# debbiemarkslab/EVcouplings

Measured on NVIDIA H100. Metric: PLM gradient evals/s as N*L^2*q cell-ops/s, higher is better.
Workload: dtype f32 parameters/accumulation; tensor-core products as bf16 hi+lo pairs (16 mantissa bits)

## Files before the change

evcouplings_b200/csrc/plm_tc.cu:

```cuda
#include <cuda.h>
#include <cuda_bf16.h>

#include <stdlib.h>

#include <algorithm>

#include "common.cuh"
#include "internal.h"

namespace evc {

constexpr int TC_BM = 128;
constexpr int TC_BN = 192;
constexpr int TC_BK = 64;
constexpr int TC_MAX_STAGES = 8;
constexpr int TC_A_BYTES = TC_BM * TC_BK * 2;
constexpr int TC_B_BYTES = TC_BN * TC_BK * 2;
constexpr int TC_SMEM_LIMIT = 232448;
constexpr int TC_SMEM_HEAD = 2048;
constexpr int TC_THREADS = 384;
constexpr int TC_CONSUMERS = 256;
constexpr int TC_K_CHUNK = 32;
constexpr int TC_MAX_KSPLIT = 8;
constexpr int TC_REG_PRODUCER = 40;
// ... 104 lines not shown
          "+f"(d[56]), "+f"(d[57]), "+f"(d[58]), "+f"(d[59]), "+f"(d[60]), "+f"(d[61]), "+f"(d[62]), "+f"(d[63]),
          "+f"(d[64]), "+f"(d[65]), "+f"(d[66]), "+f"(d[67]), "+f"(d[68]), "+f"(d[69]), "+f"(d[70]), "+f"(d[71]),
          "+f"(d[72]), "+f"(d[73]), "+f"(d[74]), "+f"(d[75]), "+f"(d[76]), "+f"(d[77]), "+f"(d[78]), "+f"(d[79]),
          "+f"(d[80]), "+f"(d[81]), "+f"(d[82]), "+f"(d[83]), "+f"(d[84]), "+f"(d[85]), "+f"(d[86]), "+f"(d[87]),
          "+f"(d[88]), "+f"(d[89]), "+f"(d[90]), "+f"(d[91]), "+f"(d[92]), "+f"(d[93]), "+f"(d[94]), "+f"(d[95])
        : "l"(da), "l"(db), "r"(scale_d));
}
template <>
__device__ __forceinline__ void wgmma_bf16<176>(float *d, uint64_t da, uint64_t db, uint32_t scale_d)
{
    asm volatile(
        "{\n.reg .pred p;\n"
        "setp.ne.b32 p, %90, 0;\n"
        "wgmma.mma_async.sync.aligned.m64n176k16.f32.bf16.bf16 "
        "{"
        "%0, %1, %2, %3, %4, %5, %6, %7, %8, %9, %10, %11, %12, %13, %14, %15, "
        "%16, %17, %18, %19, %20, %21, %22, %23, %24, %25, %26, %27, %28, %29, %30, %31, "
        "%32, %33, %34, %35, %36, %37, %38, %39, %40, %41, %42, %43, %44, %45, %46, %47, "
        "%48, %49, %50, %51, %52, %53, %54, %55, %56, %57, %58, %59, %60, %61, %62, %63, "
        "%64, %65, %66, %67, %68, %69, %70, %71, %72, %73, %74, %75, %76, %77, %78, %79, "
        "%80, %81, %82, %83, %84, %85, %86, %87"
        "}, %88, %89, p, 1, 1, 0, 0;\n}\n"
        : "+f"(d[0]), "+f"(d[1]), "+f"(d[2]), "+f"(d[3]), "+f"(d[4]), "+f"(d[5]), "+f"(d[6]), "+f"(d[7]),
          "+f"(d[8]), "+f"(d[9]), "+f"(d[10]), "+f"(d[11]), "+f"(d[12]), "+f"(d[13]), "+f"(d[14]), "+f"(d[15]),
          "+f"(d[16]), "+f"(d[17]), "+f"(d[18]), "+f"(d[19]), "+f"(d[20]), "+f"(d[21]), "+f"(d[22]), "+f"(d[23]),
          "+f"(d[24]), "+f"(d[25]), "+f"(d[26]), "+f"(d[27]), "+f"(d[28]), "+f"(d[29]), "+f"(d[30]), "+f"(d[31]),
          "+f"(d[32]), "+f"(d[33]), "+f"(d[34]), "+f"(d[35]), "+f"(d[36]), "+f"(d[37]), "+f"(d[38]), "+f"(d[39]),
          "+f"(d[40]), "+f"(d[41]), "+f"(d[42]), "+f"(d[43]), "+f"(d[44]), "+f"(d[45]), "+f"(d[46]), "+f"(d[47]),
          "+f"(d[48]), "+f"(d[49]), "+f"(d[50]), "+f"(d[51]), "+f"(d[52]), "+f"(d[53]), "+f"(d[54]), "+f"(d[55]),
          "+f"(d[56]), "+f"(d[57]), "+f"(d[58]), "+f"(d[59]), "+f"(d[60]), "+f"(d[61]), "+f"(d[62]), "+f"(d[63]),
          "+f"(d[64]), "+f"(d[65]), "+f"(d[66]), "+f"(d[67]), "+f"(d[68]), "+f"(d[69]), "+f"(d[70]), "+f"(d[71]),
          "+f"(d[72]), "+f"(d[73]), "+f"(d[74]), "+f"(d[75]), "+f"(d[76]), "+f"(d[77]), "+f"(d[78]), "+f"(d[79]),
          "+f"(d[80]), "+f"(d[81]), "+f"(d[82]), "+f"(d[83]), "+f"(d[84]), "+f"(d[85]), "+f"(d[86]), "+f"(d[87])
        : "l"(da), "l"(db), "r"(scale_d));
}

__device__ __forceinline__ void wgmma_sp_bf16_192(float *d, const uint4 &a, uint32_t e, uint64_t db, uint32_t scale_d)
{
    asm volatile(
        "{\n.reg .pred p;\n"
        "setp.ne.b32 p, %102, 0;\n"
        "wgmma.mma_async.sp.sync.aligned.m64n192k32.f32.bf16.bf16 "
        "{"
        "%0, %1, %2, %3, %4, %5, %6, %7, %8, %9, %10, %11, %12, %13, %14, %15, "
        "%16, %17, %18, %19, %20, %21, %22, %23, %24, %25, %26, %27, %28, %29, %30, %31, "
        "%32, %33, %34, %35, %36, %37, %38, %39, %40, %41, %42, %43, %44, %45, %46, %47, "
        "%48, %49, %50, %51, %52, %53, %54, %55, %56, %57, %58, %59, %60, %61, %62, %63, "
        "%64, %65, %66, %67, %68, %69, %70, %71, %72, %73, %74, %75, %76, %77, %78, %79, "
        "%80, %81, %82, %83, %84, %85, %86, %87, %88, %89, %90, %91, %92, %93, %94, %95"
        "}, {%96, %97, %98, %99}, %100, %101, 0, p, 1, 1, 0;\n}\n"
        : "+f"(d[0]), "+f"(d[1]), "+f"(d[2]), "+f"(d[3]), "+f"(d[4]), "+f"(d[5]), "+f"(d[6]), "+f"(d[7]),
          "+f"(d[8]), "+f"(d[9]), "+f"(d[10]), "+f"(d[11]), "+f"(d[12]), "+f"(d[13]), "+f"(d[14]), "+f"(d[15]),
          "+f"(d[16]), "+f"(d[17]), "+f"(d[18]), "+f"(d[19]), "+f"(d[20]), "+f"(d[21]), "+f"(d[22]), "+f"(d[23]),
          "+f"(d[24]), "+f"(d[25]), "+f"(d[26]), "+f"(d[27]), "+f"(d[28]), "+f"(d[29]), "+f"(d[30]), "+f"(d[31]),
          "+f"(d[32]), "+f"(d[33]), "+f"(d[34]), "+f"(d[35]), "+f"(d[36]), "+f"(d[37]), "+f"(d[38]), "+f"(d[39]),
          "+f"(d[40]), "+f"(d[41]), "+f"(d[42]), "+f"(d[43]), "+f"(d[44]), "+f"(d[45]), "+f"(d[46]), "+f"(d[47]),
          "+f"(d[48]), "+f"(d[49]), "+f"(d[50]), "+f"(d[51]), "+f"(d[52]), "+f"(d[53]), "+f"(d[54]), "+f"(d[55]),
          "+f"(d[56]), "+f"(d[57]), "+f"(d[58]), "+f"(d[59]), "+f"(d[60]), "+f"(d[61]), "+f"(d[62]), "+f"(d[63]),
          "+f"(d[64]), "+f"(d[65]), "+f"(d[66]), "+f"(d[67]), "+f"(d[68]), "+f"(d[69]), "+f"(d[70]), "+f"(d[71]),
          "+f"(d[72]), "+f"(d[73]), "+f"(d[74]), "+f"(d[75]), "+f"(d[76]), "+f"(d[77]), "+f"(d[78]), "+f"(d[79]),
          "+f"(d[80]), "+f"(d[81]), "+f"(d[82]), "+f"(d[83]), "+f"(d[84]), "+f"(d[85]), "+f"(d[86]), "+f"(d[87]),
          "+f"(d[88]), "+f"(d[89]), "+f"(d[90]), "+f"(d[91]), "+f"(d[92]), "+f"(d[93]), "+f"(d[94]), "+f"(d[95])
        : "r"(a.x), "r"(a.y), "r"(a.z), "r"(a.w), "l"(db), "r"(e), "r"(scale_d));
}

__device__ __forceinline__ uint4 lds128(uint32_t addr)
{
    uint4 v;
    asm volatile("ld.shared.v4.u32 {%0, %1, %2, %3}, [%4];" : "=r"(v.x), "=r"(v.y), "=r"(v.z), "=r"(v.w) : "r"(addr));
    return v;
}
__device__ __forceinline__ uint32_t lds32(uint32_t addr)
{
    uint32_t v;
    asm volatile("ld.shared.u32 %0, [%1];" : "=r"(v) : "r"(addr));
    return v;
}
__device__ __forceinline__ uint32_t cluster_ctarank()
{
    uint32_t r;
    asm volatile("mov.u32 %0, %%cluster_ctarank;" : "=r"(r));
    return r;
}
__device__ __forceinline__ void cluster_sync()
{
    asm volatile("barrier.cluster.arrive.release;\nbarrier.cluster.wait.acquire;" ::: "memory");
}
__device__ __forceinline__ void mbar_arrive_cluster(uint64_t *bar, uint32_t rank)
{
    uint32_t remote;
    asm volatile("mapa.shared::cluster.u32 %0, %1, %2;" : "=r"(remote) : "r"(smem_u32(bar)), "r"(rank));
    asm volatile("mbarrier.arrive.shared::cluster.b64 _, [%0];" ::"r"(remote) : "memory");
}
__device__ __forceinline__ void tma_load_2d_multicast(void *smem_dst, const CUtensorMap *tmap, int c0, int c1,
                                                      uint64_t *bar, uint16_t mask, uint64_t policy)
{
    asm volatile(
        "cp.async.bulk.tensor.2d.shared::cluster.global.mbarrier::complete_tx::bytes.multicast::cluster.L2::cache_hint"
        " [%0], [%1, {%4, %5}], [%2], %3, %6;"
        ::"r"(smem_u32(smem_dst)), "l"(reinterpret_cast<uint64_t>(tmap)), "r"(smem_u32(bar)), "h"(mask), "r"(c0),
        "r"(c1), "l"(policy)
        : "memory");
}

template <int N>
__device__ __forceinline__ void wgmma_kblock(float *acc, uint64_t a, uint64_t b, uint64_t a2, uint64_t b2, bool two,
                                             bool overwrite)
{
#pragma unroll
    for (int k = 0; k < TC_BK / 16; k++) {
        const uint64_t koff = (uint64_t)((k * 16 * 2) >> 4);
        wgmma_bf16<N>(acc, a + koff, b + koff, (overwrite && k == 0) ? 0u : 1u);
        if (two) wgmma_bf16<N>(acc, a2 + koff, b2 + koff, 1u);
    }
}

template <int N>
__device__ __forceinline__ void tc_mainloop(float *acc, uint64_t *full, uint64_t *empty, int &s, uint32_t &ph,
                                            int n_stages, int stage_bytes, int kb0, int kb1, uint64_t desc0,
                                            uint64_t off_a, uint64_t off_b, uint64_t off_a2, uint64_t off_b2, bool two)
{
    int prev = -1;
    for (int kb = kb0; kb < kb1; kb++) {
        mbar_wait_bounded(&full[s], ph);
        wgmma_fence();
        const uint64_t d = desc0 + (uint64_t)((s * stage_bytes) >> 4);
        wgmma_kblock<N>(acc, d + off_a, d + off_b, d + off_a2, d + off_b2, two, kb == kb0);
        wgmma_commit();
        wgmma_wait<1>();
        if (prev >= 0) mbar_arrive(&empty[prev]);
        prev = s;
        if (++s == n_stages) { s = 0; ph ^= 1u; }
    }
    wgmma_wait<0>();
    fence_regs<N / 2>(acc);
    if (prev >= 0) mbar_arrive(&empty[prev]);
}

__device__ __forceinline__ void decode_tile(int tile, int m_tiles, int n_tiles, int mgroup, int &m_tile, int &n_tile)
{
    const int full = (m_tiles / mgroup) * mgroup * n_tiles;
    if (tile < full) {
        const int per = mgroup * n_tiles;
        const int g = tile / per, r = tile - g * per;
        n_tile = r / mgroup;
        m_tile = g * mgroup + (r - n_tile * mgroup);
    } else {
        const int rem = m_tiles % mgroup, r = tile - full;
        n_tile = r / rem;
        m_tile = (m_tiles / mgroup) * mgroup + (r - n_tile * rem);
    }
}

struct TcSmem {
    uint64_t *full, *empty;
    unsigned char *ring;
};
__device__ __forceinline__ TcSmem tc_smem_layout(unsigned char *smem_dyn)
{
    unsigned char *base = reinterpret_cast<unsigned char *>((reinterpret_cast<uintptr_t>(smem_dyn) + 1023) &
                                                            ~static_cast<uintptr_t>(1023));
    TcSmem l;
    l.full = reinterpret_cast<uint64_t *>(base);
    l.empty = l.full + TC_MAX_STAGES;
    l.ring = base + 1024;
    return l;
// ... 23 lines not shown
    extern __shared__ unsigned char smem_dyn[];
    const TcSmem l = tc_smem_layout(smem_dyn);
    const int tiles = m_tiles * n_tiles;
    const int slice = (int)blockIdx.x / tiles;
    int m_tile, n_tile;
    decode_tile((int)blockIdx.x - slice * tiles, m_tiles, n_tiles, mgroup, m_tile, n_tile);
    const int kb_per = (num_kb + ksplit - 1) / ksplit;
    const int kb_begin = slice * kb_per, kb_end = min(num_kb, kb_begin + kb_per);
    tc_init_barriers(l, n_stages);

    if (threadIdx.x < 128) {
        setmaxnreg_dec<TC_REG_PRODUCER>();
        if (threadIdx.x == 0) {
            int s = 0;
            uint32_t ph = 0;
            for (int kb = kb_begin; kb < kb_end; kb++) {
                mbar_wait_bounded(&l.empty[s], ph ^ 1u);
                unsigned char *st = l.ring + s * stage_bytes;
                mbar_expect_tx(&l.full[s], (uint32_t)stage_bytes);
                tma_load_2d(st, &tm0, kb * TC_BK, m_tile * TC_BM, &l.full[s]);
                tma_load_2d(st + BYTES0, &tm1, kb * TC_BK, n_tile * TC_BN, &l.full[s]);
                if (!SINGLE) tma_load_2d(st + BYTES0 + BYTES1, &tm2, kb * TC_BK, n_tile * TC_BN, &l.full[s]);
                if (++s == n_stages) { s = 0; ph ^= 1u; }
            }
        }
    } else {
        setmaxnreg_inc<TC_REG_CONSUMER>();
        const int cw = (threadIdx.x >> 7) - 1;
        constexpr uint64_t OFF1 = (uint64_t)(BYTES0 >> 4), OFF2 = (uint64_t)((BYTES0 + BYTES1) >> 4);
        const uint64_t arow = (uint64_t)((cw * 64 * TC_BK * 2) >> 4);
        const uint64_t desc0 = make_desc_sw128(l.ring);
        float acc[TC_BN / 2], sum[TC_BN / 2];
#pragma unroll
        for (int u = 0; u < TC_BN / 2; u++) acc[u] = 0.f;
        const int n_chunks = (kb_end - kb_begin + k_chunk - 1) / k_chunk;
        int s = 0;
        uint32_t ph = 0;
        for (int c = 0; c < n_chunks; c++) {
            const int kb0 = kb_begin + c * k_chunk, kb1 = min(kb_end, kb0 + k_chunk);
            tc_mainloop<TC_BN>(acc, l.full, l.empty, s, ph, n_stages, stage_bytes, kb0, kb1, desc0,
                               arow, OFF1, arow, OFF2, !SINGLE);
#pragma unroll
            for (int u = 0; u < TC_BN / 2; u++) sum[u] = (c == 0) ? acc[u] : sum[u] + acc[u];
        }
        const int t = threadIdx.x & 127;
        const int64_t row = (int64_t)m_tile * TC_BM + cw * 64 + (t >> 5) * 16 + ((t & 31) >> 2);
        float *out = D + slice * plane + row * ldd + (int64_t)n_tile * TC_BN + 2 * (t & 3);
        if (ACC && slice < acc_planes) {
#pragma unroll
            for (int c8 = 0; c8 < TC_BN / 8; c8++) {
                float2 *p0 = reinterpret_cast<float2 *>(out + 8 * c8);
                float2 *p1 = reinterpret_cast<float2 *>(out + 8 * ldd + 8 * c8);
                const float2 v0 = __ldcs(p0), v1 = __ldcs(p1);
                __stcs(p0, make_float2(v0.x + sum[4 * c8], v0.y + sum[4 * c8 + 1]));
                __stcs(p1, make_float2(v1.x + sum[4 * c8 + 2], v1.y + sum[4 * c8 + 3]));
            }
            return;
        }
#pragma unroll
        for (int c8 = 0; c8 < TC_BN / 8; c8++) {
            __stcs(reinterpret_cast<float2 *>(out + 8 * c8), make_float2(sum[4 * c8], sum[4 * c8 + 1]));
            __stcs(reinterpret_cast<float2 *>(out + 8 * ldd + 8 * c8), make_float2(sum[4 * c8 + 2], sum[4 * c8 + 3]));
        }
    }
}

constexpr int XSP_STEP_BYTES = 2560;
constexpr int XSP_KB_BYTES = 4 * XSP_STEP_BYTES;
constexpr int SP_W_HALF = (TC_BN / 2) * TC_BK * 2;

template <int SINGLE, int PAIR>
__global__ void __launch_bounds__(TC_THREADS, 1)
tc_sparse_logits_kernel(const __grid_constant__ CUtensorMap tm_hi, const __grid_constant__ CUtensorMap tm_lo,
                        const unsigned char *__restrict__ xsp, float *__restrict__ Zt, int64_t ldz, int64_t rows_z,
                        int state_tiles, int seq_tiles, int seq_units, int num_kb, int k_chunk, int group,
                        int n_stages)
{
    constexpr int TILES = PAIR ? 2 : 1;
    constexpr int OFF_A = TC_B_BYTES;
    constexpr int OFF_LO = TC_B_BYTES + TILES * XSP_KB_BYTES;
    constexpr int stage_bytes = OFF_LO + (SINGLE ? 0 : TC_B_BYTES);
    extern __shared__ unsigned char smem_dyn[];
    const TcSmem l = tc_smem_layout(smem_dyn);
    uint32_t cs;
    asm volatile("mov.u32 %0, %%cluster_nctarank;" : "=r"(cs));
    const uint32_t rank = cluster_ctarank();
    int n_tile, unit;
    decode_tile((int)(blockIdx.x / cs), state_tiles, seq_units, group, n_tile, unit);
    const int seq_tile0 = (unit * (int)cs + (int)rank) * TILES;
    if (threadIdx.x == 0) {
        for (int s = 0; s < n_stages; s++) {
            mbar_init(&l.full[s], 1);
            mbar_init(&l.empty[s], 8 * cs);
        }
        mbar_fence_init();
    }
    cluster_sync();

    if (threadIdx.x < 128) {
        setmaxnreg_dec<PAIR ? TC_REG_PRODUCER_PAIR : TC_REG_PRODUCER>();
        if (threadIdx.x == 0) {
            const uint64_t keep = l2_policy_evict_last();
            const unsigned char *src[TILES];
#pragma unroll
            for (int i = 0; i < TILES; i++) {
                const int tile = seq_tile0 + i;
                src[i] = xsp + (int64_t)(tile >= seq_tiles ? 0 : tile) * num_kb * XSP_KB_BYTES;
            }
            const int row0 = n_tile * TC_BN;
            int s = 0;
            uint32_t ph = 0;
            for (int kb = 0; kb < num_kb; kb++) {
                mbar_wait_bounded(&l.empty[s], ph ^ 1u);
                unsigned char *st = l.ring + s * stage_bytes;
                mbar_expect_tx(&l.full[s], (uint32_t)stage_bytes);
#pragma unroll
                for (int i = 0; i < TILES; i++)
                    bulk_g2s(st + OFF_A + i * XSP_KB_BYTES, src[i] + (int64_t)kb * XSP_KB_BYTES, XSP_KB_BYTES,
                             &l.full[s]);
                if (cs == 1) {
                    for (int h = 0; h < 2; h++) {
                        tma_load_2d_hint(st + h * SP_W_HALF, &tm_hi, kb * TC_BK, row0 + h * (TC_BN / 2), &l.full[s], keep);
                        if (!SINGLE)
                            tma_load_2d_hint(st + OFF_LO + h * SP_W_HALF, &tm_lo, kb * TC_BK, row0 + h * (TC_BN / 2),
                                             &l.full[s], keep);
                    }
                } else {
                    const int h = (int)rank;
                    tma_load_2d_multicast(st + h * SP_W_HALF, &tm_hi, kb * TC_BK, row0 + h * (TC_BN / 2), &l.full[s],
                                          (uint16_t)0x3, keep);
                    if (!SINGLE)
                        tma_load_2d_multicast(st + OFF_LO + h * SP_W_HALF, &tm_lo, kb * TC_BK, row0 + h * (TC_BN / 2),
                                              &l.full[s], (uint16_t)0x3, keep);
                }
                if (++s == n_stages) { s = 0; ph ^= 1u; }
            }
        }
    } else {
        setmaxnreg_inc<PAIR ? TC_REG_CONSUMER_PAIR : TC_REG_CONSUMER>();
        const int cw = (threadIdx.x >> 7) - 1;
        const int t = threadIdx.x & 127;
        const uint32_t a_addr = smem_u32(l.ring) + OFF_A + cw * (PAIR ? XSP_KB_BYTES : 2 * XSP_STEP_BYTES) + 16 * t;
        const uint32_t e_addr = a_addr + 2048 - 12 * t;
        const uint64_t desc0 = make_desc_sw128(l.ring);
        constexpr uint64_t DLO = (uint64_t)(OFF_LO >> 4), DK32 = (uint64_t)((32 * 2) >> 4);
        auto release = [&](int st) {
            if ((threadIdx.x & 31) == 0) {
                mbar_arrive_cluster(&l.empty[st], 0);
                if (cs == 2) mbar_arrive_cluster(&l.empty[st], 1);
            }
        };
        auto store = [&](const float *const *v, int nb, int tile, int rb) {
            if (tile >= seq_tiles) return;
            const int64_t seq0 = (int64_t)tile * TC_BM + rb + (t >> 5) * 16 + ((t & 31) >> 2);
            const int64_t st0 = (int64_t)n_tile * TC_BN + 2 * (t & 3);
            bool col[2][2];
#pragma unroll
            for (int b = 0; b < 2; b++)
#pragma unroll
                for (int h = 0; h < 2; h++) col[b][h] = b < nb && seq0 + 64 * b + 8 * h < ldz;
            const int64_t nrows = rows_z - st0;
            float *p = Zt + st0 * ldz + seq0;
#pragma unroll
            for (int c8 = 0; c8 < TC_BN / 8; c8++) {
#pragma unroll
                for (int e = 0; e < 4; e++)
#pragma unroll
                    for (int b = 0; b < 2; b++)
                        if (8 * c8 + (e & 1) < nrows && col[b][e >> 1])
                            __stcs(p + (e & 1) * ldz + 64 * b + 8 * (e >> 1), v[b][4 * c8 + e]);
                p += 8 * ldz;
            }
        };
        if (PAIR) {
            float acc0[TC_BN / 2], acc1[TC_BN / 2];
#pragma unroll
            for (int u = 0; u < TC_BN / 2; u++) acc0[u] = acc1[u] = 0.f;
            int s = 0;
            uint32_t ph = 0;
            for (int kb = 0; kb < num_kb; kb++) {
                mbar_wait_bounded(&l.full[s], ph);
                const uint32_t so = (uint32_t)(s * stage_bytes);
                const uint4 a00 = lds128(a_addr + so), a01 = lds128(a_addr + so + XSP_STEP_BYTES);
                const uint4 a10 = lds128(a_addr + so + 2 * XSP_STEP_BYTES), a11 = lds128(a_addr + so + 3 * XSP_STEP_BYTES);
                const uint32_t e00 = lds32(e_addr + so), e01 = lds32(e_addr + so + XSP_STEP_BYTES);
                const uint32_t e10 = lds32(e_addr + so + 2 * XSP_STEP_BYTES), e11 = lds32(e_addr + so + 3 * XSP_STEP_BYTES);
                wgmma_fence();
                const uint64_t d = desc0 + (uint64_t)((s * stage_bytes) >> 4);
                const uint32_t sc = kb == 0 ? 0u : 1u;
                wgmma_sp_bf16_192(acc0, a00, e00, d, sc);
                wgmma_sp_bf16_192(acc1, a10, e10, d, sc);
                if (!SINGLE) {
                    wgmma_sp_bf16_192(acc0, a00, e00, d + DLO, 1u);
                    wgmma_sp_bf16_192(acc1, a10, e10, d + DLO, 1u);
                }
                wgmma_sp_bf16_192(acc0, a01, e01, d + DK32, 1u);
                wgmma_sp_bf16_192(acc1, a11, e11, d + DK32, 1u);
                if (!SINGLE) {
                    wgmma_sp_bf16_192(acc0, a01, e01, d + DLO + DK32, 1u);
                    wgmma_sp_bf16_192(acc1, a11, e11, d + DLO + DK32, 1u);
                }
                wgmma_commit();
                wgmma_wait<0>();
                release(s);
                if (++s == n_stages) { s = 0; ph ^= 1u; }
            }
            fence_regs<TC_BN / 2>(acc0);
            fence_regs<TC_BN / 2>(acc1);
            const float *v[2] = {acc0, acc1};
            store(v, 2, seq_tile0 + cw, 0);
        } else {
            float acc[TC_BN / 2], sum[TC_BN / 2];
#pragma unroll
            for (int u = 0; u < TC_BN / 2; u++) acc[u] = 0.f;
            const int n_chunks = (num_kb + k_chunk - 1) / k_chunk;
            int s = 0;
            uint32_t ph = 0;
            for (int c = 0; c < n_chunks; c++) {
                const int kb0 = c * k_chunk, kb1 = min(num_kb, kb0 + k_chunk);
                for (int kb = kb0; kb < kb1; kb++) {
                    mbar_wait_bounded(&l.full[s], ph);
                    const uint32_t so = (uint32_t)(s * stage_bytes);
                    const uint4 a0 = lds128(a_addr + so), a1 = lds128(a_addr + so + XSP_STEP_BYTES);
                    const uint32_t e0 = lds32(e_addr + so), e1 = lds32(e_addr + so + XSP_STEP_BYTES);
                    wgmma_fence();
                    const uint64_t d = desc0 + (uint64_t)((s * stage_bytes) >> 4);
                    wgmma_sp_bf16_192(acc, a0, e0, d, kb == kb0 ? 0u : 1u);
                    if (!SINGLE) wgmma_sp_bf16_192(acc, a0, e0, d + DLO, 1u);
                    wgmma_sp_bf16_192(acc, a1, e1, d + DK32, 1u);
                    if (!SINGLE) wgmma_sp_bf16_192(acc, a1, e1, d + DLO + DK32, 1u);
                    wgmma_commit();
                    wgmma_wait<0>();
                    release(s);
                    if (++s == n_stages) { s = 0; ph ^= 1u; }
                }
                fence_regs<TC_BN / 2>(acc);
#pragma unroll
                for (int u = 0; u < TC_BN / 2; u++) sum[u] = (c == 0) ? acc[u] : sum[u] + acc[u];
            }
            const float *v[2] = {sum, sum};
            store(v, 1, seq_tile0, cw * 64);
        }
    }
    cluster_sync();
}

__device__ __forceinline__ uint32_t xsp_group(const uint32_t *__restrict__ msa4, int64_t Nld, int64_t n, bool real,
                                              int k, int lq, int q, uint32_t &vals)
{
    uint32_t mask = 0;
    if (real) {
#pragma unroll
        for (int p = 0; p < 4; p++) {
            const int kk = k + p;
            if (kk >= lq) break;
            const int j = kk / q, b = kk - j * q;
            const int code = (int)((msa4[(int64_t)(j >> 2) * Nld + n] >> (8 * (j & 3))) & 0xffu);
            mask |= (uint32_t)(code == b) << p;
        }
    }
    int i0 = 0, i1 = 1;
    if (__popc(mask) == 2) { i0 = __ffs(mask) - 1; i1 = 31 - __clz(mask); }
    else if (mask > 2) i1 = __ffs(mask) - 1;
    vals = (((mask >> i0) & 1u) ? 0x3F80u : 0u) | ((((mask >> i1) & 1u) ? 0x3F80u : 0u) << 16);
    return (uint32_t)(i0 | (i1 << 2));
}

__global__ void build_xsp_kernel(const uint32_t *__restrict__ msa4, unsigned char *__restrict__ out, int64_t n0,
                                 int64_t nreal, int64_t Nld, int L, int q, int num_kb, int64_t n_frag)
{
    const int64_t gt = (int64_t)blockIdx.x * blockDim.x + threadIdx.x;
    if (gt >= n_frag * 128) return;
    const int64_t ci = gt >> 7;
    const int t = (int)(gt & 127);
    const int step = (int)(ci & 1), cw = (int)((ci >> 1) & 1);
    const int64_t tkb = ci >> 2;
    const int kb = (int)(tkb % num_kb);
    const int64_t T = tkb / num_kb;
    const int64_t r0 = T * TC_BM + cw * 64 + (t >> 5) * 16 + ((t & 31) >> 2), r1 = r0 + 8;
    const int k0 = kb * TC_BK + step * 32, lq = L * q;
    const int c = t & 3, h = c & 1;
    uint32_t e = 0, v[2][2], unused;
#pragma unroll
    for (int rr = 0; rr < 2; rr++) {
        const int64_t r = rr ? r1 : r0;
#pragma unroll
        for (int i = 0; i < 4; i++)
            e |= xsp_group(msa4, Nld, n0 + r, r < nreal, k0 + 4 * (4 * h + i), lq, q, unused) << (16 * rr + 4 * i);
#pragma unroll
        for (int u = 0; u < 2; u++) xsp_group(msa4, Nld, n0 + r, r < nreal, k0 + 4 * (4 * u + c), lq, q, v[rr][u]);
    }
    unsigned char *frag = out + ci * XSP_STEP_BYTES;
    reinterpret_cast<uint4 *>(frag)[t] = make_uint4(v[0][0], v[1][0], v[0][1], v[1][1]);
    reinterpret_cast<uint32_t *>(frag + 2048)[t] = e;
}

constexpr int TF_BN = 176;
constexpr int TF_SITES = 8;
constexpr int TF_B_BYTES = TF_BN * TC_BK * 2;
constexpr int TF_PITCH = TF_BN + 1;

template <int SINGLE>
__global__ void __launch_bounds__(TC_THREADS, 1)
tc_fwd_fused_kernel(const __grid_constant__ CUtensorMap tm_x, const __grid_constant__ CUtensorMap tm_whi,
                    const __grid_constant__ CUtensorMap tm_wlo, const float *__restrict__ h,
                    const uint32_t *__restrict__ msa4, const float *__restrict__ wts,
                    __nv_bfloat16 *__restrict__ Rt_hi, __nv_bfloat16 *__restrict__ Rt_lo, int64_t Kp,
                    float *__restrict__ gh_part, double *__restrict__ fx_part, PlmGeom g, int m_tiles, int n_tiles,
                    int num_kb, int n_stages)
{
    constexpr int Q = 21;
    extern __shared__ unsigned char smem_dyn[];
    const TcSmem l = tc_smem_layout(smem_dyn);
    constexpr int stage_bytes = TC_A_BYTES + TF_B_BYTES + (SINGLE ? 0 : TF_B_BYTES);
    const int n_tile = blockIdx.x % n_tiles, m_tile = blockIdx.x / n_tiles;
    const int q = g.q;
    tc_init_barriers(l, n_stages);

    if (threadIdx.x < 128) {
        setmaxnreg_dec<TC_REG_PRODUCER>();
        if (threadIdx.x == 0) {
            const uint64_t keep = l2_policy_evict_last();
            int s = 0;
            uint32_t ph = 0;
// ... 549 lines not shown
    if (make_map(&m[0], d_wt_hi, t.Mp, t.Kw, TC_BN / 2)) return 1;
    if (make_map(&m[1], d_wt_lo, t.Mp, t.Kw, TC_BN / 2)) return 1;
    return 0;
}

int plm_tcf_build_xsp(const PlmGeom &g, const PlmTcfGeom &t, const uint32_t *d_msa4, void *d_x1h, int64_t n0,
                      cudaStream_t st)
{
    const int num_kb = (int)(t.Kw / TC_BK);
    const int64_t n_frag = t.Xrows / TC_BM * num_kb * 4;
    build_xsp_kernel<<<(unsigned)ceil_div(n_frag * 128, 256), 256, 0, st>>>(
        d_msa4, reinterpret_cast<unsigned char *>(d_x1h), n0, std::min(t.Xrows, g.N - n0), g.Nld, g.L, g.q, num_kb,
        n_frag);
    EVC_KERNEL_CHECK();
    return 0;
}

int plm_tcf_expand(const PlmGeom &g, const PlmTcfGeom &t, const float *d_x, void *d_wt_hi, void *d_wt_lo,
                   int single, cudaStream_t st)
{
    const unsigned nt = (unsigned)ceil_div(g.L, EXP_SITES);
    if (g.q > EXP_STATIC_Q) {
        const size_t smem = exp_wide_smem(g.q);
        EVC_CUDA(cudaFuncSetAttribute(expand_tc_kernel<false, true>, cudaFuncAttributeMaxDynamicSharedMemorySize,
                                      (int)smem));
        expand_tc_kernel<false, true><<<dim3(nt, nt), EXP_THREADS, smem, st>>>(
            d_x, reinterpret_cast<__nv_bfloat16 *>(d_wt_hi), reinterpret_cast<__nv_bfloat16 *>(d_wt_lo), g.L, g.q,
            t.Kw, single);
        EVC_KERNEL_CHECK();
        return 0;
    }
    expand_tc_kernel<false><<<dim3(nt, nt), EXP_THREADS, 0, st>>>(d_x, reinterpret_cast<__nv_bfloat16 *>(d_wt_hi),
                                                                  reinterpret_cast<__nv_bfloat16 *>(d_wt_lo), g.L, g.q,
                                                                  t.Kw, single);
    EVC_KERNEL_CHECK();
    return 0;
}

static int forward_group(const PlmTcfGeom &t, int single, int tiles)
{
    static int mg_env = -2;
    const int e = env_int_once("EVC_MGROUP", &mg_env);
    if (e > 0) return std::min(e, tiles);
    static int mb_env = -2;
    const int mb = env_int_once("EVC_MGROUP_MB", &mb_env);
    const double budget = (mb > 0 ? mb : 24) * 1.0e6;
    const double per_tile = (double)TC_BN * (double)t.Kw * 2.0 * (single ? 1.0 : 2.0);
    return std::max(1, std::min(tiles, (int)(budget / per_tile)));
}

static int forward_cluster()
{
    static int cl_env = -2;
    const int e = env_int_once("EVC_FWD_CLUSTER", &cl_env);
    return e == 1 ? 1 : 2;
}

static bool forward_pair(int num_kb, int kchunk)
{
    static int tile_env = -2;
    const int e = env_int_once("EVC_FWD_TILE", &tile_env);
    return e != 128 && kchunk >= num_kb;
}

int plm_tcf_logits(const PlmGeom &g, const PlmTcfGeom &t, const void *maps, const void *d_x1h, float *d_zt,
                   int single, int64_t nreal, cudaStream_t st)
{
    const CUtensorMap *m = reinterpret_cast<const CUtensorMap *>(maps);
    const int num_kb = (int)(t.Kw / TC_BK);
    const int kchunk = num_kb <= 128 ? num_kb : TC_K_CHUNK;
    const bool pair = forward_pair(num_kb, kchunk);
    const int stage = TC_B_BYTES + (pair ? 2 : 1) * XSP_KB_BYTES + (single ? 0 : TC_B_BYTES);
    const int n_stages = stages_for(stage);
    const size_t smem = (size_t)n_stages * stage + TC_SMEM_HEAD;
    const int cs = forward_cluster();
    const int state_tiles = (int)ceil_div((int64_t)g.L * g.q, TC_BN);
    const int seq_tiles = (int)ceil_div(nreal, TC_BM);
    const int seq_units = (int)ceil_div(ceil_div(seq_tiles, pair ? 2 : 1), cs);
    const int group = forward_group(t, single, state_tiles);
    auto kernel = pair ? (single ? tc_sparse_logits_kernel<1, 1> : tc_sparse_logits_kernel<0, 1>)
                       : (single ? tc_sparse_logits_kernel<1, 0> : tc_sparse_logits_kernel<0, 0>);
    EVC_CUDA(cudaFuncSetAttribute(kernel, cudaFuncAttributeMaxDynamicSharedMemorySize, TC_SMEM_LIMIT));
    cudaLaunchConfig_t cfg = {};
    cfg.gridDim = dim3((unsigned)(state_tiles * seq_units * cs));
    cfg.blockDim = dim3(TC_THREADS);
    cfg.dynamicSmemBytes = smem;
    cfg.stream = st;
    cudaLaunchAttribute attr[1];
    attr[0].id = cudaLaunchAttributeClusterDimension;
    attr[0].val.clusterDim.x = (unsigned)cs;
    attr[0].val.clusterDim.y = 1;
    attr[0].val.clusterDim.z = 1;
    cfg.attrs = attr;
    cfg.numAttrs = 1;
    EVC_CUDA(cudaLaunchKernelEx(&cfg, kernel, m[0], m[1], reinterpret_cast<const unsigned char *>(d_x1h), d_zt, t.Ns,
                                t.Mp, state_tiles, seq_tiles, seq_units, num_kb, kchunk, group, n_stages));
    EVC_KERNEL_CHECK();
    return 0;
}

template <bool ONEHOT>
static int launch_softmax(const PlmGeom &g, int ntiles, const float *d_zt, int64_t ldz, const float *d_x,
                          const uint32_t *d_msa4, const float *d_wts, __nv_bfloat16 *hi, __nv_bfloat16 *lo,
                          int64_t Kp, float *d_gh_part, double *d_fx_part, int64_t n0, int64_t nreal, cudaStream_t st)
{
    dim3 grid((unsigned)ceil_div(nreal, 256), (unsigned)g.L);
    switch (g.q) {
        case 21: plm_softmax_kernel<21, ONEHOT><<<grid, 128, 0, st>>>(d_zt, ldz, d_x, d_msa4, d_wts, hi, lo, Kp, d_gh_part, d_fx_part, g, ntiles, n0); break;
        case 20: plm_softmax_kernel<20, ONEHOT><<<grid, 128, 0, st>>>(d_zt, ldz, d_x, d_msa4, d_wts, hi, lo, Kp, d_gh_part, d_fx_part, g, ntiles, n0); break;
        case 5: plm_softmax_kernel<5, ONEHOT><<<grid, 128, 0, st>>>(d_zt, ldz, d_x, d_msa4, d_wts, hi, lo, Kp, d_gh_part, d_fx_part, g, ntiles, n0); break;
        case 4: plm_softmax_kernel<4, ONEHOT><<<grid, 128, 0, st>>>(d_zt, ldz, d_x, d_msa4, d_wts, hi, lo, Kp, d_gh_part, d_fx_part, g, ntiles, n0); break;
        default:
            if (g.q < 2 || g.q > PLM_MAX_Q) { set_error("plm softmax kernel: unsupported q"); return 1; }
            if (g.q <= 8)
                plm_softmax_kernel<8, ONEHOT, true><<<grid, 128, 0, st>>>(d_zt, ldz, d_x, d_msa4, d_wts, hi, lo, Kp, d_gh_part, d_fx_part, g, ntiles, n0);
            else if (g.q <= 16)
                plm_softmax_kernel<16, ONEHOT, true><<<grid, 128, 0, st>>>(d_zt, ldz, d_x, d_msa4, d_wts, hi, lo, Kp, d_gh_part, d_fx_part, g, ntiles, n0);
            else
                plm_softmax_kernel<32, ONEHOT, true><<<grid, 128, 0, st>>>(d_zt, ldz, d_x, d_msa4, d_wts, hi, lo, Kp, d_gh_part, d_fx_part, g, ntiles, n0);
    }
    EVC_KERNEL_CHECK();
    return 0;
}

int plm_tcf_softmax(const PlmGeom &g, const PlmTcfGeom &t, const float *d_zt, const float *d_x,
                    const uint32_t *d_msa4, const float *d_wts, void *d_rt_hi, void *d_rt_lo, int64_t Kp,
                    float *d_gh_part, double *d_fx_part, int64_t n0, int64_t nreal, cudaStream_t st)
{
    return launch_softmax<false>(g, t.ntiles_s, d_zt, t.Ns, d_x, d_msa4, d_wts,
                                 reinterpret_cast<__nv_bfloat16 *>(d_rt_hi), reinterpret_cast<__nv_bfloat16 *>(d_rt_lo),
                                 Kp, d_gh_part, d_fx_part, n0, nreal, st);
}

int plm_tc_onehot_residual(const PlmGeom &g, int ntiles, const uint32_t *d_msa4, const float *d_wts, void *d_rt_hi,
                           void *d_rt_lo, int64_t Kp, float *d_gh_part, double *d_fx_part, int64_t n0, int64_t nreal,
                           cudaStream_t st)
{
    return launch_softmax<true>(g, ntiles, nullptr, 0, nullptr, d_msa4, d_wts,
                                reinterpret_cast<__nv_bfloat16 *>(d_rt_hi), reinterpret_cast<__nv_bfloat16 *>(d_rt_lo),
                                Kp, d_gh_part, d_fx_part, n0, nreal, st);
}

void plm_tcff_geometry(const PlmGeom &g, PlmTcffGeom &t)
{
    t.n_tiles = (int)ceil_div(g.L, TF_SITES);
    t.Np = (int64_t)t.n_tiles * TF_BN;
    t.Kw = round_up((int64_t)g.L * g.q, TC_BK);
    t.m_tiles = (int)ceil_div(g.N, TC_BM);
    t.Xrows = round_up(g.N, 384);
    t.ntile_part = t.m_tiles * 4;
}

bool plm_tcff_supported(const PlmGeom &g) { return g.S == 21; }

int plm_tcff_make_maps(const PlmTcffGeom &t, void *d_x1h, void *d_wp_hi, void *d_wp_lo, void *maps_out)
{
    CUtensorMap *m = reinterpret_cast<CUtensorMap *>(maps_out);
    if (make_map(&m[0], d_x1h, t.Xrows, t.Kw, TC_BM)) return 1;
    if (make_map(&m[1], d_wp_hi, t.Np, t.Kw, TF_BN)) return 1;
    if (make_map(&m[2], d_wp_lo, t.Np, t.Kw, TF_BN)) return 1;
    return 0;
}

int plm_tcff_expand(const PlmGeom &g, const PlmTcffGeom &t, const float *d_x, void *d_wp_hi, void *d_wp_lo,
                    int single, cudaStream_t st)
{
    const unsigned nt = (unsigned)ceil_div(g.L, EXP_SITES);
    expand_tc_kernel<true><<<dim3(nt, nt), EXP_THREADS, 0, st>>>(d_x, reinterpret_cast<__nv_bfloat16 *>(d_wp_hi),
                                                                 reinterpret_cast<__nv_bfloat16 *>(d_wp_lo), g.L, g.q,
                                                                 t.Kw, single);
    EVC_KERNEL_CHECK();
    return 0;
}

int plm_tcff_forward(const PlmGeom &g, const PlmTcffGeom &t, const void *maps, const float *d_x,
                     const uint32_t *d_msa4, const float *d_wts, void *d_rt_hi, void *d_rt_lo, int64_t Kp,
                     float *d_gh_part, double *d_fx_part, int single, cudaStream_t st)
// ... 19 lines not shown
```

Before: 5272 billion.

## Make sparse logits forward kernel persistent over tile units

After: 5303 billion, median of 6. About the same (+0.6%).

```diff
diff --git a/evcouplings_b200/csrc/plm_tc.cu b/evcouplings_b200/csrc/plm_tc.cu
--- a/evcouplings_b200/csrc/plm_tc.cu
+++ b/evcouplings_b200/csrc/plm_tc.cu
@@ -210,6 +210,12 @@
     asm volatile("mov.u32 %0, %%cluster_ctarank;" : "=r"(r));
     return r;
 }
+__device__ __forceinline__ uint32_t cluster_nctarank()
+{
+    uint32_t r;
+    asm volatile("mov.u32 %0, %%cluster_nctarank;" : "=r"(r));
+    return r;
+}
 __device__ __forceinline__ void cluster_sync()
 {
     asm volatile("barrier.cluster.arrive.release;\nbarrier.cluster.wait.acquire;" ::: "memory");
@@ -399,62 +405,72 @@
     constexpr int stage_bytes = OFF_LO + (SINGLE ? 0 : TC_B_BYTES);
     extern __shared__ unsigned char smem_dyn[];
     const TcSmem l = tc_smem_layout(smem_dyn);
-    uint32_t cs;
-    asm volatile("mov.u32 %0, %%cluster_nctarank;" : "=r"(cs));
-    const uint32_t rank = cluster_ctarank();
-    int n_tile, unit;
-    decode_tile((int)(blockIdx.x / cs), state_tiles, seq_units, group, n_tile, unit);
-    const int seq_tile0 = (unit * (int)cs + (int)rank) * TILES;
     if (threadIdx.x == 0) {
         for (int s = 0; s < n_stages; s++) {
             mbar_init(&l.full[s], 1);
-            mbar_init(&l.empty[s], 8 * cs);
+            mbar_init(&l.empty[s], 8 * cluster_nctarank());
         }
         mbar_fence_init();
     }
     cluster_sync();
+    const int units = state_tiles * seq_units;
+    auto cluster_geometry = [&](uint32_t &cs, uint32_t &rank, int &cluster, int &n_clusters) {
+        cs = cluster_nctarank();
+        rank = cluster_ctarank();
+        cluster = (int)(blockIdx.x / cs);
+        n_clusters = (int)(gridDim.x / cs);
+    };
+    uint32_t cs, rank;
+    int cluster, n_clusters;
 
     if (threadIdx.x < 128) {
         setmaxnreg_dec<PAIR ? TC_REG_PRODUCER_PAIR : TC_REG_PRODUCER>();
-        if (threadIdx.x == 0) {
-            const uint64_t keep = l2_policy_evict_last();
-            const unsigned char *src[TILES];
-#pragma unroll
-            for (int i = 0; i < TILES; i++) {
-                const int tile = seq_tile0 + i;
-                src[i] = xsp + (int64_t)(tile >= seq_tiles ? 0 : tile) * num_kb * XSP_KB_BYTES;
-            }
-            const int row0 = n_tile * TC_BN;
+        cluster_geometry(cs, rank, cluster, n_clusters);
+        if (threadIdx.x < 32) {
+            const bool issue = threadIdx.x == 0;
             int s = 0;
             uint32_t ph = 0;
-            for (int kb = 0; kb < num_kb; kb++) {
-                mbar_wait_bounded(&l.empty[s], ph ^ 1u);
-                unsigned char *st = l.ring + s * stage_bytes;
-                mbar_expect_tx(&l.full[s], (uint32_t)stage_bytes);
-#pragma unroll
-                for (int i = 0; i < TILES; i++)
-                    bulk_g2s(st + OFF_A + i * XSP_KB_BYTES, src[i] + (int64_t)kb * XSP_KB_BYTES, XSP_KB_BYTES,
-                             &l.full[s]);
-                if (cs == 1) {
-                    for (int h = 0; h < 2; h++) {
-                        tma_load_2d_hint(st + h * SP_W_HALF, &tm_hi, kb * TC_BK, row0 + h * (TC_BN / 2), &l.full[s], keep);
-                        if (!SINGLE)
-                            tma_load_2d_hint(st + OFF_LO + h * SP_W_HALF, &tm_lo, kb * TC_BK, row0 + h * (TC_BN / 2),
-                                             &l.full[s], keep);
+            for (int u = cluster; u < units; u += n_clusters) {
+                int n_tile, unit;
+                decode_tile(u, state_tiles, seq_units, group, n_tile, unit);
+                const int seq_tile0 = (unit * (int)cs + (int)rank) * TILES;
+                const int row0 = n_tile * TC_BN;
+                const unsigned char *src = xsp + (int64_t)(seq_tile0 < seq_tiles ? seq_tile0 : 0) * num_kb * XSP_KB_BYTES;
+                const int64_t next = seq_tile0 + 1 < seq_tiles ? (int64_t)num_kb * XSP_KB_BYTES : xsp - src;
+                for (int kb = 0; kb < num_kb; kb++, src += XSP_KB_BYTES) {
+                    mbar_wait_bounded(&l.empty[s], ph ^ 1u);
+                    if (issue) {
+                        const uint64_t keep = l2_policy_evict_last();
+                        unsigned char *st = l.ring + s * stage_bytes;
+                        mbar_expect_tx(&l.full[s], (uint32_t)stage_bytes);
+#pragma unroll
+                        for (int i = 0; i < TILES; i++)
+                            bulk_g2s(st + OFF_A + i * XSP_KB_BYTES, i ? src + next : src, XSP_KB_BYTES, &l.full[s]);
+                        if (cs == 1) {
+                            for (int h = 0; h < 2; h++) {
+                                tma_load_2d_hint(st + h * SP_W_HALF, &tm_hi, kb * TC_BK, row0 + h * (TC_BN / 2),
+                                                 &l.full[s], keep);
+                                if (!SINGLE)
+                                    tma_load_2d_hint(st + OFF_LO + h * SP_W_HALF, &tm_lo, kb * TC_BK,
+                                                     row0 + h * (TC_BN / 2), &l.full[s], keep);
+                            }
+                        } else {
+                            const int h = (int)rank;
+                            tma_load_2d_multicast(st + h * SP_W_HALF, &tm_hi, kb * TC_BK, row0 + h * (TC_BN / 2),
+                                                  &l.full[s], (uint16_t)0x3, keep);
+                            if (!SINGLE)
+                                tma_load_2d_multicast(st + OFF_LO + h * SP_W_HALF, &tm_lo, kb * TC_BK,
+                                                      row0 + h * (TC_BN / 2), &l.full[s], (uint16_t)0x3, keep);
+                        }
                     }
-                } else {
-                    const int h = (int)rank;
-                    tma_load_2d_multicast(st + h * SP_W_HALF, &tm_hi, kb * TC_BK, row0 + h * (TC_BN / 2), &l.full[s],
-                                          (uint16_t)0x3, keep);
-                    if (!SINGLE)
-                        tma_load_2d_multicast(st + OFF_LO + h * SP_W_HALF, &tm_lo, kb * TC_BK, row0 + h * (TC_BN / 2),
-                                              &l.full[s], (uint16_t)0x3, keep);
+                    __syncwarp();
+                    if (++s == n_stages) { s = 0; ph ^= 1u; }
                 }
-                if (++s == n_stages) { s = 0; ph ^= 1u; }
             }
         }
     } else {
         setmaxnreg_inc<PAIR ? TC_REG_CONSUMER_PAIR : TC_REG_CONSUMER>();
+        cluster_geometry(cs, rank, cluster, n_clusters);
         const int cw = (threadIdx.x >> 7) - 1;
         const int t = threadIdx.x & 127;
         const uint32_t a_addr = smem_u32(l.ring) + OFF_A + cw * (PAIR ? XSP_KB_BYTES : 2 * XSP_STEP_BYTES) + 16 * t;
@@ -467,7 +483,7 @@
                 if (cs == 2) mbar_arrive_cluster(&l.empty[st], 1);
             }
         };
-        auto store = [&](const float *const *v, int nb, int tile, int rb) {
+        auto store = [&](const float *const *v, int nb, int n_tile, int tile, int rb) {
             if (tile >= seq_tiles) return;
             const int64_t seq0 = (int64_t)tile * TC_BM + rb + (t >> 5) * 16 + ((t & 31) >> 2);
             const int64_t st0 = (int64_t)n_tile * TC_BN + 2 * (t & 3);
@@ -489,74 +505,80 @@
                 p += 8 * ldz;
             }
         };
+        int s = 0;
+        uint32_t ph = 0;
         if (PAIR) {
             float acc0[TC_BN / 2], acc1[TC_BN / 2];
 #pragma unroll
             for (int u = 0; u < TC_BN / 2; u++) acc0[u] = acc1[u] = 0.f;
-            int s = 0;
-            uint32_t ph = 0;
-            for (int kb = 0; kb < num_kb; kb++) {
-                mbar_wait_bounded(&l.full[s], ph);
-                const uint32_t so = (uint32_t)(s * stage_bytes);
-                const uint4 a00 = lds128(a_addr + so), a01 = lds128(a_addr + so + XSP_STEP_BYTES);
-                const uint4 a10 = lds128(a_addr + so + 2 * XSP_STEP_BYTES), a11 = lds128(a_addr + so + 3 * XSP_STEP_BYTES);
-                const uint32_t e00 = lds32(e_addr + so), e01 = lds32(e_addr + so + XSP_STEP_BYTES);
-                const uint32_t e10 = lds32(e_addr + so + 2 * XSP_STEP_BYTES), e11 = lds32(e_addr + so + 3 * XSP_STEP_BYTES);
-                wgmma_fence();
-                const uint64_t d = desc0 + (uint64_t)((s * stage_bytes) >> 4);
-                const uint32_t sc = kb == 0 ? 0u : 1u;
-                wgmma_sp_bf16_192(acc0, a00, e00, d, sc);
-                wgmma_sp_bf16_192(acc1, a10, e10, d, sc);
-                if (!SINGLE) {
-                    wgmma_sp_bf16_192(acc0, a00, e00, d + DLO, 1u);
-                    wgmma_sp_bf16_192(acc1, a10, e10, d + DLO, 1u);
-                }
-                wgmma_sp_bf16_192(acc0, a01, e01, d + DK32, 1u);
-                wgmma_sp_bf16_192(acc1, a11, e11, d + DK32, 1u);
-                if (!SINGLE) {
-                    wgmma_sp_bf16_192(acc0, a01, e01, d + DLO + DK32, 1u);
-                    wgmma_sp_bf16_192(acc1, a11, e11, d + DLO + DK32, 1u);
-                }
-                wgmma_commit();
-                wgmma_wait<0>();
-                release(s);
-                if (++s == n_stages) { s = 0; ph ^= 1u; }
-            }
-            fence_regs<TC_BN / 2>(acc0);
-            fence_regs<TC_BN / 2>(acc1);
-            const float *v[2] = {acc0, acc1};
-            store(v, 2, seq_tile0 + cw, 0);
-        } else {
-            float acc[TC_BN / 2], sum[TC_BN / 2];
-#pragma unroll
-            for (int u = 0; u < TC_BN / 2; u++) acc[u] = 0.f;
-            const int n_chunks = (num_kb + k_chunk - 1) / k_chunk;
-            int s = 0;
-            uint32_t ph = 0;
-            for (int c = 0; c < n_chunks; c++) {
-                const int kb0 = c * k_chunk, kb1 = min(num_kb, kb0 + k_chunk);
-                for (int kb = kb0; kb < kb1; kb++) {
+            for (int u = cluster; u < units; u += n_clusters) {
+                int n_tile, unit;
+                decode_tile(u, state_tiles, seq_units, group, n_tile, unit);
+                for (int kb = 0; kb < num_kb; kb++) {
                     mbar_wait_bounded(&l.full[s], ph);
                     const uint32_t so = (uint32_t)(s * stage_bytes);
-                    const uint4 a0 = lds128(a_addr + so), a1 = lds128(a_addr + so + XSP_STEP_BYTES);
-                    const uint32_t e0 = lds32(e_addr + so), e1 = lds32(e_addr + so + XSP_STEP_BYTES);
+                    const uint4 a00 = lds128(a_addr + so), a01 = lds128(a_addr + so + XSP_STEP_BYTES);
+                    const uint4 a10 = lds128(a_addr + so + 2 * XSP_STEP_BYTES), a11 = lds128(a_addr + so + 3 * XSP_STEP_BYTES);
+                    const uint32_t e00 = lds32(e_addr + so), e01 = lds32(e_addr + so + XSP_STEP_BYTES);
+                    const uint32_t e10 = lds32(e_addr + so + 2 * XSP_STEP_BYTES), e11 = lds32(e_addr + so + 3 * XSP_STEP_BYTES);
                     wgmma_fence();
                     const uint64_t d = desc0 + (uint64_t)((s * stage_bytes) >> 4);
-                    wgmma_sp_bf16_192(acc, a0, e0, d, kb == kb0 ? 0u : 1u);
-                    if (!SINGLE) wgmma_sp_bf16_192(acc, a0, e0, d + DLO, 1u);
-                    wgmma_sp_bf16_192(acc, a1, e1, d + DK32, 1u);
-                    if (!SINGLE) wgmma_sp_bf16_192(acc, a1, e1, d + DLO + DK32, 1u);
+                    const uint32_t sc = kb == 0 ? 0u : 1u;
+                    wgmma_sp_bf16_192(acc0, a00, e00, d, sc);
+                    wgmma_sp_bf16_192(acc1, a10, e10, d, sc);
+                    if (!SINGLE) {
+                        wgmma_sp_bf16_192(acc0, a00, e00, d + DLO, 1u);
+                        wgmma_sp_bf16_192(acc1, a10, e10, d + DLO, 1u);
+                    }
+                    wgmma_sp_bf16_192(acc0, a01, e01, d + DK32, 1u);
+                    wgmma_sp_bf16_192(acc1, a11, e11, d + DK32, 1u);
+                    if (!SINGLE) {
+                        wgmma_sp_bf16_192(acc0, a01, e01, d + DLO + DK32, 1u);
+                        wgmma_sp_bf16_192(acc1, a11, e11, d + DLO + DK32, 1u);
+                    }
                     wgmma_commit();
                     wgmma_wait<0>();
                     release(s);
                     if (++s == n_stages) { s = 0; ph ^= 1u; }
                 }
-                fence_regs<TC_BN / 2>(acc);
-#pragma unroll
-                for (int u = 0; u < TC_BN / 2; u++) sum[u] = (c == 0) ? acc[u] : sum[u] + acc[u];
+                fence_regs<TC_BN / 2>(acc0);
+                fence_regs<TC_BN / 2>(acc1);
+                const float *v[2] = {acc0, acc1};
+                store(v, 2, n_tile, (unit * (int)cs + (int)rank) * TILES + cw, 0);
             }
-            const float *v[2] = {sum, sum};
-            store(v, 1, seq_tile0, cw * 64);
+        } else {
+            float acc[TC_BN / 2], sum[TC_BN / 2];
+#pragma unroll
+            for (int u = 0; u < TC_BN / 2; u++) acc[u] = 0.f;
+            const int n_chunks = (num_kb + k_chunk - 1) / k_chunk;
+            for (int u = cluster; u < units; u += n_clusters) {
+                int n_tile, unit;
+                decode_tile(u, state_tiles, seq_units, group, n_tile, unit);
+                for (int c = 0; c < n_chunks; c++) {
+                    const int kb0 = c * k_chunk, kb1 = min(num_kb, kb0 + k_chunk);
+                    for (int kb = kb0; kb < kb1; kb++) {
+                        mbar_wait_bounded(&l.full[s], ph);
+                        const uint32_t so = (uint32_t)(s * stage_bytes);
+                        const uint4 a0 = lds128(a_addr + so), a1 = lds128(a_addr + so + XSP_STEP_BYTES);
+                        const uint32_t e0 = lds32(e_addr + so), e1 = lds32(e_addr + so + XSP_STEP_BYTES);
+                        wgmma_fence();
+                        const uint64_t d = desc0 + (uint64_t)((s * stage_bytes) >> 4);
+                        wgmma_sp_bf16_192(acc, a0, e0, d, kb == kb0 ? 0u : 1u);
+                        if (!SINGLE) wgmma_sp_bf16_192(acc, a0, e0, d + DLO, 1u);
+                        wgmma_sp_bf16_192(acc, a1, e1, d + DK32, 1u);
+                        if (!SINGLE) wgmma_sp_bf16_192(acc, a1, e1, d + DLO + DK32, 1u);
+                        wgmma_commit();
+                        wgmma_wait<0>();
+                        release(s);
+                        if (++s == n_stages) { s = 0; ph ^= 1u; }
+                    }
+                    fence_regs<TC_BN / 2>(acc);
+#pragma unroll
+                    for (int i = 0; i < TC_BN / 2; i++) sum[i] = (c == 0) ? acc[i] : sum[i] + acc[i];
+                }
+                const float *v[2] = {sum, sum};
+                store(v, 1, n_tile, unit * (int)cs + (int)rank, cw * 64);
+            }
         }
     }
     cluster_sync();
@@ -1272,7 +1294,6 @@
                        : (single ? tc_sparse_logits_kernel<1, 0> : tc_sparse_logits_kernel<0, 0>);
     EVC_CUDA(cudaFuncSetAttribute(kernel, cudaFuncAttributeMaxDynamicSharedMemorySize, TC_SMEM_LIMIT));
     cudaLaunchConfig_t cfg = {};
-    cfg.gridDim = dim3((unsigned)(state_tiles * seq_units * cs));
     cfg.blockDim = dim3(TC_THREADS);
     cfg.dynamicSmemBytes = smem;
     cfg.stream = st;
@@ -1283,6 +1304,15 @@
     attr[0].val.clusterDim.z = 1;
     cfg.attrs = attr;
     cfg.numAttrs = 1;
+    static int resident[2][2][2] = {};
+    int &fit = resident[pair ? 1 : 0][single ? 1 : 0][cs - 1];
+    if (fit == 0) {
+        cfg.gridDim = dim3((unsigned)cs);
+        EVC_CUDA(cudaOccupancyMaxActiveClusters(&fit, kernel, &cfg));
+        if (fit <= 0) { set_error("sparse forward: no cluster of the forward kernel fits on the device"); return 1; }
+    }
+    const int units = state_tiles * seq_units;
+    cfg.gridDim = dim3((unsigned)(std::min(units, fit) * cs));
     EVC_CUDA(cudaLaunchKernelEx(&cfg, kernel, m[0], m[1], reinterpret_cast<const unsigned char *>(d_x1h), d_zt, t.Ns,
                                 t.Mp, state_tiles, seq_tiles, seq_units, num_kb, kchunk, group, n_stages));
     EVC_KERNEL_CHECK();
```
